# joshbeal/mira

Hardware: AMD Instinct MI355X
Metric: bn256_g1_msm_throughput (higher is better)
Workload: dtype u256 mod p (9 x 29-bit limbs in u32/u64, Montgomery)

## Files before the change

mira_amd/csrc/field29.cuh:

```cuda
#pragma once
#include "field.cuh"

struct Fq29 {
    using Sat = FqP;
    static constexpr uint32_t P[9] = {0x187cfd47u, 0x010460b6u, 0x1c72a34fu, 0x02d522d0u, 0x1585d978u, 0x02db40c0u, 0x00a6e141u, 0x0e5c2634u, 0x0030644eu};
    static constexpr uint32_t N0 = 0x04866389u;
    static constexpr uint32_t ONE[9] = {0x157ccc21u, 0x141c2758u, 0x185230d3u, 0x014c0419u, 0x0aa36fb9u, 0x1d4240ceu, 0x11d54c07u, 0x052ac7a8u, 0x000dc836u};
    static constexpr uint32_t R256_TO_R261[9] = {0x13349ca1u, 0x1a5d84a8u, 0x0a3e5cacu, 0x100249e0u, 0x12b951e8u, 0x0e92d304u, 0x14cb95b3u, 0x041b9d3du, 0x00058003u};
};
struct Fr29 {
    using Sat = FrP;
    static constexpr uint32_t P[9] = {0x10000001u, 0x1f0fac9fu, 0x0e5c2450u, 0x07d090f3u, 0x1585d283u, 0x02db40c0u, 0x00a6e141u, 0x0e5c2634u, 0x0030644eu};
    static constexpr uint32_t N0 = 0x0fffffffu;
    static constexpr uint32_t ONE[9] = {0x0fffff57u, 0x1ea70ab4u, 0x052c068bu, 0x17504f49u, 0x0aa8075bu, 0x1d4240ceu, 0x11d54c07u, 0x052ac7a8u, 0x000dc836u};
    static constexpr uint32_t R256_TO_R261[9] = {0x0fffead7u, 0x1d5444f4u, 0x04438aa5u, 0x03b4d096u, 0x134c84dau, 0x0e92d304u, 0x14cb95b3u, 0x041b9d3du, 0x00058003u};
};

static constexpr uint32_t M29 = 0x1FFFFFFFu;

#ifdef F29_TRACK
#include <cassert>
#include "f29_census.h"
#define F29_BD(x) double bd = (x);
#define F29_SET(v, x) ((v).bd = (x))
#define F29_GET(v) ((v).bd)
#define F29_ASSERT(c) assert(c)
#define F29_HIT(fn, site) emu_hit(fn, site)
#define F29_REGION(name) EMU_REGION_SCOPE(name)
#else
#define F29_BD(x)
#define F29_SET(v, x) ((void)0)
#define F29_GET(v) (0.0)
#define F29_ASSERT(c) ((void)0)
#define F29_HIT(fn, site) ((void)0)
#define F29_REGION(name) ((void)0)
#endif
static constexpr double F29_RP_OVER_P = 168.0;

template <class F> struct Fe29 {
    uint32_t l[9];
    F29_BD(0.0)
};

template <class F> HD Fe29<F> f29_zero() {
    Fe29<F> r;
#pragma unroll
    for (int i = 0; i < 9; i++) r.l[i] = 0;
    return r;
}
template <class F> HD Fe29<F> f29_one() {
    Fe29<F> r;
#pragma unroll
    for (int i = 0; i < 9; i++) r.l[i] = F::ONE[i];
    F29_SET(r, 1.0);
    return r;
}
template <class F> HD bool f29_is_literal_zero(const Fe29<F> &a) {
    uint32_t o = 0;
#pragma unroll
    for (int i = 0; i < 9; i++) o |= a.l[i];
    return o == 0;
}

template <class F> HD Fe29<F> f29_carry(const Fe29<F> &a) {
    Fe29<F> r;
    r.l[0] = a.l[0] & M29;
#pragma unroll
    for (int i = 1; i < 8; i++) r.l[i] = (a.l[i] & M29) + (a.l[i - 1] >> 29);
    r.l[8] = a.l[8] + (a.l[7] >> 29);
    F29_SET(r, F29_GET(a));
    return r;
}
template <class F> HD Fe29<F> f29_add(const Fe29<F> &a, const Fe29<F> &b) {
    Fe29<F> r;
#pragma unroll
    for (int i = 0; i < 9; i++) r.l[i] = a.l[i] + b.l[i];
    F29_SET(r, F29_GET(a) + F29_GET(b));
    F29_ASSERT(F29_GET(r) <= 40.0);
    return f29_carry(r);
}
template <class F> HD Fe29<F> f29_dbl(const Fe29<F> &a) { return f29_add(a, a); }
template <class F, int K> struct F29Bias {
    uint32_t l[9];
    constexpr F29Bias() : l{} {
        uint64_t carry = 0;
        for (int i = 0; i < 9; i++) {
            uint64_t v = (uint64_t)K * F::P[i] + carry;
            l[i] = (i < 8) ? (uint32_t)(v & M29) : (uint32_t)v;
            carry = v >> 29;
        }
        for (int i = 0; i < 8; i++) {
            l[i] += 0x80000000u;
            l[i + 1] -= 4;
        }
    }
};
template <int K, class F> HD Fe29<F> f29_sub(const Fe29<F> &a, const Fe29<F> &b) {
    constexpr F29Bias<F, K> bias{};
    Fe29<F> r;
#pragma unroll
    for (int i = 0; i < 9; i++) r.l[i] = a.l[i] + bias.l[i] - b.l[i];
    F29_ASSERT(F29_GET(b) <= (double)K - 0.01);
    F29_SET(r, F29_GET(a) + (double)K);
    F29_ASSERT(F29_GET(r) <= 40.0);
    return f29_carry(r);
}
template <int K, class F> HD Fe29<F> f29_sub_b_2c(const Fe29<F> &a, const Fe29<F> &b, const Fe29<F> &c) {
    constexpr F29Bias<F, K> bias{};
    Fe29<F> r;
#pragma unroll
    for (int i = 0; i < 9; i++) r.l[i] = a.l[i] + bias.l[i] - b.l[i] - 2u * c.l[i];
    F29_ASSERT(F29_GET(b) + 2.0 * F29_GET(c) <= (double)K - 0.01);
    F29_SET(r, F29_GET(a) + (double)K);
    F29_ASSERT(F29_GET(r) <= 40.0);
    return f29_carry(r);
}
template <int K, class F> HD Fe29<F> f29_neg(const Fe29<F> &b) { return f29_sub<K>(f29_zero<F>(), b); }
template <class F> HD Fe29<F> f29_triple(const Fe29<F> &a) { return f29_add(f29_dbl(a), a); }

template <class F> HD Fe29<F> f29_add_nc(const Fe29<F> &a, const Fe29<F> &b) {
    Fe29<F> r;
#pragma unroll
    for (int i = 0; i < 9; i++) r.l[i] = a.l[i] + b.l[i];
    F29_SET(r, F29_GET(a) + F29_GET(b));
    F29_ASSERT(F29_GET(r) <= 40.0);
    return r;
}
template <class F, int K, int RAISE = 1> struct F29BiasTight {
    uint32_t l[9];
    bool ok;
    constexpr F29BiasTight() : l{}, ok(true) {
        uint64_t carry = 0;
        for (int i = 0; i < 9; i++) {
            uint64_t v = (uint64_t)K * F::P[i] + carry;
            l[i] = (i < 8) ? (uint32_t)(v & M29) : (uint32_t)v;
            carry = v >> 29;
            if (l[i] < 8u) ok = false;
        }
        for (int i = 0; i < 8; i++) {
            l[i] += (uint32_t)RAISE * 0x20000000u;
            l[i + 1] -= (uint32_t)RAISE;
        }
    }
};
template <int K, class F, int RAISE = 1> HD Fe29<F> f29_sub_nc(const Fe29<F> &a, const Fe29<F> &b) {
    constexpr F29BiasTight<F, K, RAISE> bias{};
    static_assert(bias.ok, "a limb of K * P is too small for this bias");
    Fe29<F> r;
#pragma unroll
    for (int i = 0; i < 9; i++) {
        F29_ASSERT(b.l[i] <= bias.l[i]);
        r.l[i] = a.l[i] + bias.l[i] - b.l[i];
        F29_ASSERT(r.l[i] >= a.l[i]);
    }
    F29_ASSERT(F29_GET(b) <= (double)K - 1.0);
    F29_SET(r, F29_GET(a) + (double)K);
    F29_ASSERT(F29_GET(r) <= 40.0);
    return r;
}
#ifdef F29_TRACK
template <class F> inline void f29_check_columns(const Fe29<F> &a, const Fe29<F> &b) {
    uint32_t ma = 0, mb = 0;
    for (int i = 0; i < 9; i++) { ma = a.l[i] > ma ? a.l[i] : ma; mb = b.l[i] > mb ? b.l[i] : mb; }
    const long double col = 9.0L * (long double)ma * (long double)mb + 9.0L * 536870912.0L * 536870912.0L + 68719476736.0L;
    assert(col < 18446744073709551616.0L);
}
template <class F> inline void f29_check_columns2(const Fe29<F> &a, const Fe29<F> &b, const Fe29<F> &c, const Fe29<F> &d) {
    uint32_t m[4] = {0, 0, 0, 0};
    const Fe29<F> *v[4] = {&a, &b, &c, &d};
    for (int k = 0; k < 4; k++)
        for (int i = 0; i < 9; i++) m[k] = v[k]->l[i] > m[k] ? v[k]->l[i] : m[k];
    const long double col = 9.0L * ((long double)m[0] * m[1] + (long double)m[2] * m[3]) + 9.0L * 536870912.0L * 536870912.0L + 68719476736.0L;
    assert(col < 18446744073709551616.0L);
}
#define F29_CHECK_COLUMNS(a, b) f29_check_columns(a, b)
#define F29_CHECK_COLUMNS2(a, b, c, d) f29_check_columns2(a, b, c, d)
#else
#define F29_CHECK_COLUMNS(a, b) ((void)0)
#define F29_CHECK_COLUMNS2(a, b, c, d) ((void)0)
#endif

template <class F> HD Fe29<F> f29_mul(const Fe29<F> &a, const Fe29<F> &b) {
    F29_ASSERT(F29_GET(a) * F29_GET(b) <= F29_RP_OVER_P);
    F29_CHECK_COLUMNS(a, b);
    uint64_t c[18];
#pragma unroll
    for (int k = 0; k < 18; k++) c[k] = 0;
#pragma unroll
    for (int i = 0; i < 9; i++)
#pragma unroll
        for (int j = 0; j < 9; j++) c[i + j] += (uint64_t)a.l[i] * b.l[j];
#pragma unroll
    for (int k = 0; k < 9; k++) {
        uint32_t m = ((uint32_t)c[k] * F::N0) & M29;
#pragma unroll
        for (int j = 0; j < 9; j++) c[k + j] += (uint64_t)m * F::P[j];
        c[k + 1] += c[k] >> 29;
    }
    Fe29<F> r;
#pragma unroll
    for (int i = 9; i < 17; i++) {
        r.l[i - 9] = (uint32_t)c[i] & M29;
        c[i + 1] += c[i] >> 29;
    }
    r.l[8] = (uint32_t)c[17];
    F29_SET(r, F29_GET(a) * F29_GET(b) / 168.9 + 1.0);
    return r;
}
template <class F> HD Fe29<F> f29_mul2_add(const Fe29<F> &a, const Fe29<F> &b, const Fe29<F> &c2, const Fe29<F> &d) {
    F29_ASSERT(F29_GET(a) * F29_GET(b) + F29_GET(c2) * F29_GET(d) <= F29_RP_OVER_P);
    F29_CHECK_COLUMNS2(a, b, c2, d);
    uint64_t c[18];
#pragma unroll
    for (int k = 0; k < 18; k++) c[k] = 0;
#pragma unroll
    for (int i = 0; i < 9; i++)
#pragma unroll
        for (int j = 0; j < 9; j++) c[i + j] += (uint64_t)a.l[i] * b.l[j];
#pragma unroll
    for (int i = 0; i < 9; i++)
#pragma unroll
        for (int j = 0; j < 9; j++) c[i + j] += (uint64_t)c2.l[i] * d.l[j];
#pragma unroll
    for (int k = 0; k < 9; k++) {
        uint32_t m = ((uint32_t)c[k] * F::N0) & M29;
#pragma unroll
        for (int j = 0; j < 9; j++) c[k + j] += (uint64_t)m * F::P[j];
        c[k + 1] += c[k] >> 29;
    }
    Fe29<F> r;
#pragma unroll
    for (int i = 9; i < 17; i++) {
        r.l[i - 9] = (uint32_t)c[i] & M29;
        c[i + 1] += c[i] >> 29;
    }
    r.l[8] = (uint32_t)c[17];
    F29_SET(r, (F29_GET(a) * F29_GET(b) + F29_GET(c2) * F29_GET(d)) / 168.9 + 1.0);
    return r;
}
template <class F> HD Fe29<F> f29_redc(const Fe29<F> &a) {
    uint64_t c[18];
#pragma unroll
    for (int k = 0; k < 9; k++) { c[k] = a.l[k]; c[k + 9] = 0; }
#pragma unroll
    for (int k = 0; k < 9; k++) {
        uint32_t m = ((uint32_t)c[k] * F::N0) & M29;
#pragma unroll
        for (int j = 0; j < 9; j++) c[k + j] += (uint64_t)m * F::P[j];
        c[k + 1] += c[k] >> 29;
    }
    Fe29<F> r;
#pragma unroll
    for (int i = 9; i < 17; i++) {
        r.l[i - 9] = (uint32_t)c[i] & M29;
        c[i + 1] += c[i] >> 29;
    }
    r.l[8] = (uint32_t)c[17];
    F29_SET(r, F29_GET(a) / 168.9 + 1.0);
    return r;
}
template <class F> HD Fe29<F> f29_sqr(const Fe29<F> &a) {
    F29_ASSERT(F29_GET(a) * F29_GET(a) <= F29_RP_OVER_P);
    uint64_t c[18];
#pragma unroll
    for (int k = 0; k < 18; k++) c[k] = 0;
    uint32_t d[9];
#pragma unroll
    for (int i = 0; i < 9; i++) d[i] = a.l[i] << 1;
#pragma unroll
    for (int i = 0; i < 9; i++) {
        c[2 * i] += (uint64_t)a.l[i] * a.l[i];
#pragma unroll
        for (int j = i + 1; j < 9; j++) c[i + j] += (uint64_t)a.l[i] * d[j];
    }
#pragma unroll
    for (int k = 0; k < 9; k++) {
        uint32_t m = ((uint32_t)c[k] * F::N0) & M29;
#pragma unroll
        for (int j = 0; j < 9; j++) c[k + j] += (uint64_t)m * F::P[j];
        c[k + 1] += c[k] >> 29;
    }
    Fe29<F> r;
#pragma unroll
    for (int i = 9; i < 17; i++) {
        r.l[i - 9] = (uint32_t)c[i] & M29;
        c[i + 1] += c[i] >> 29;
    }
    r.l[8] = (uint32_t)c[17];
    F29_SET(r, F29_GET(a) * F29_GET(a) / 168.9 + 1.0);
    return r;
}

constexpr uint32_t f29_inv_mod_2_29(uint32_t p0) {
    uint32_t x = p0;
    for (int i = 0; i < 5; i++) x *= 2u - p0 * x;
    return x & M29;
}
template <int KMAX, class F> HD bool f29_is_zero_mod_p(const Fe29<F> &a) {
    F29_ASSERT(F29_GET(a) <= (double)KMAX);
    constexpr uint32_t PINV = f29_inv_mod_2_29(F::P[0]);
    static_assert(((F::P[0] * PINV) & M29) == 1u, "P[0]^-1 mod 2^29");
    const bool maybe = ((a.l[0] * PINV) & M29) <= (uint32_t)KMAX;
    if (!maybe) return false;
    uint32_t n[9];
    uint32_t carry = 0;
#pragma unroll
    for (int i = 0; i < 8; i++) {
        uint32_t v = a.l[i] + carry;
        n[i] = v & M29;
        carry = v >> 29;
    }
    n[8] = a.l[8] + carry;
    for (uint32_t k = 0; k <= KMAX; k++) {
        uint64_t cy = 0;
        bool eq = true;
#pragma unroll
        for (int i = 0; i < 9; i++) {
            cy += (uint64_t)k * F::P[i];
            uint32_t want = (i < 8) ? (uint32_t)(cy & M29) : (uint32_t)cy;
            cy >>= 29;
            eq &= (n[i] == want);
        }
        if (eq) return true;
    }
    return false;
}

template <class F> HD Fe29<F> f29_unpack(const Fe<typename F::Sat> &s) {
    Fe29<F> r;
    r.l[0] = s.l[0] & M29;
    r.l[1] = ((s.l[0] >> 29) | (s.l[1] << 3)) & M29;
    r.l[2] = ((s.l[1] >> 26) | (s.l[2] << 6)) & M29;
    r.l[3] = ((s.l[2] >> 23) | (s.l[3] << 9)) & M29;
    r.l[4] = ((s.l[3] >> 20) | (s.l[4] << 12)) & M29;
    r.l[5] = ((s.l[4] >> 17) | (s.l[5] << 15)) & M29;
    r.l[6] = ((s.l[5] >> 14) | (s.l[6] << 18)) & M29;
    r.l[7] = ((s.l[6] >> 11) | (s.l[7] << 21)) & M29;
    r.l[8] = s.l[7] >> 8;
    F29_SET(r, 6.0);
    return r;
}
template <class F> HD Fe29<F> f29_unpack_canonical(const Fe<typename F::Sat> &s) {
    Fe29<F> r = f29_unpack<F>(s);
    F29_SET(r, 1.0);
    return r;
}
template <class F> HD Fe<typename F::Sat> f29_pack(const Fe29<F> &a) {
    uint32_t n[9];
    uint32_t carry = 0;
#pragma unroll
    for (int i = 0; i < 8; i++) {
        uint32_t v = a.l[i] + carry;
        n[i] = v & M29;
        carry = v >> 29;
    }
    n[8] = a.l[8] + carry;
    Fe<typename F::Sat> s;
    s.l[0] = n[0] | (n[1] << 29);
    s.l[1] = (n[1] >> 3) | (n[2] << 26);
    s.l[2] = (n[2] >> 6) | (n[3] << 23);
    s.l[3] = (n[3] >> 9) | (n[4] << 20);
    s.l[4] = (n[4] >> 12) | (n[5] << 17);
    s.l[5] = (n[5] >> 15) | (n[6] << 14);
    s.l[6] = (n[6] >> 18) | (n[7] << 11);
    s.l[7] = (n[7] >> 21) | (n[8] << 8);
    return s;
}
template <class F> HD Fe<typename F::Sat> f29_pack_product(const Fe29<F> &a) {
#pragma unroll
    for (int i = 0; i < 8; i++) F29_ASSERT(a.l[i] <= M29);
    Fe<typename F::Sat> s;
    s.l[0] = a.l[0] | (a.l[1] << 29);
    s.l[1] = (a.l[1] >> 3) | (a.l[2] << 26);
    s.l[2] = (a.l[2] >> 6) | (a.l[3] << 23);
    s.l[3] = (a.l[3] >> 9) | (a.l[4] << 20);
    s.l[4] = (a.l[4] >> 12) | (a.l[5] << 17);
    s.l[5] = (a.l[5] >> 15) | (a.l[6] << 14);
    s.l[6] = (a.l[6] >> 18) | (a.l[7] << 11);
    s.l[7] = (a.l[7] >> 21) | (a.l[8] << 8);
    return s;
}
template <class F> HD Fe29<F> f29_from_r256(const Fe<typename F::Sat> &s) {
    Fe29<F> k;
#pragma unroll
    for (int i = 0; i < 9; i++) k.l[i] = F::R256_TO_R261[i];
    F29_SET(k, 1.0);
    return f29_mul(f29_unpack_canonical<F>(s), k);
}
template <class F> HD Fe<typename F::Sat> f29_to_r256(const Fe29<F> &a) {
    Fe<typename F::Sat> r1;
#pragma unroll
    for (int i = 0; i < 8; i++) r1.l[i] = F::Sat::R1[i];
    Fe29<F> v = f29_mul(a, f29_unpack_canonical<F>(r1));
    Fe<typename F::Sat> s = f29_pack(v);
    return reduce_once(s);
}
```

mira_amd/csrc/graph_jit.hip:

```cpp
#include "ctx.h"
#include "graph_jit.hpp"
#ifndef MIRA_CPU_EMU
#include <dlfcn.h>
#include <fcntl.h>
#include <sys/stat.h>
#include <unistd.h>

#include "jit_headers.inc"
namespace graphjit {
Rtc &rtc() {
    static Rtc loaded = [] {
        Rtc r;
        for (const char *name : {"libhiprtc.so", "libhiprtc.so.7", "/opt/rocm/lib/libhiprtc.so"}) {
            r.lib = dlopen(name, RTLD_NOW | RTLD_LOCAL);
            if (r.lib) break;
        }
        if (!r.lib) { r.error = "libhiprtc.so not found: graphs stay interpreted"; return r; }
        auto sym = [&](const char *n) { void *p = dlsym(r.lib, n); if (!p) r.error = std::string("libhiprtc.so lacks ") + n; return p; };
        r.create = reinterpret_cast<decltype(r.create)>(sym("hiprtcCreateProgram"));
        r.compile = reinterpret_cast<decltype(r.compile)>(sym("hiprtcCompileProgram"));
        r.log_size = reinterpret_cast<decltype(r.log_size)>(sym("hiprtcGetProgramLogSize"));
        r.log = reinterpret_cast<decltype(r.log)>(sym("hiprtcGetProgramLog"));
        r.code_size = reinterpret_cast<decltype(r.code_size)>(sym("hiprtcGetCodeSize"));
        r.code = reinterpret_cast<decltype(r.code)>(sym("hiprtcGetCode"));
        r.destroy = reinterpret_cast<decltype(r.destroy)>(sym("hiprtcDestroyProgram"));
        return r;
    }();
    return loaded;
}
static const char *const JIT_OPTIONS[] = {"--offload-arch=gfx950", "-O3", "-std=c++17"};
std::vector<char> compile(const std::string &src, std::string &err) {
    Rtc &r = rtc();
    std::vector<char> out;
    if (!r.error.empty()) { err = r.error; return out; }
    void *prog = nullptr;
    if (r.create(&prog, src.c_str(), "mira_jit.hip", JIT_HDR_COUNT, const_cast<const char **>(JIT_HDR_TEXT), const_cast<const char **>(JIT_HDR_NAME)) != 0) {
        err = "hiprtcCreateProgram failed";
        return out;
    }
    const int rc = r.compile(prog, 3, const_cast<const char **>(JIT_OPTIONS));
    if (rc != 0) {
        size_t n = 0;
        (void)r.log_size(prog, &n);
        std::string log(n, 0);
        if (n > 1) (void)r.log(prog, &log[0]);
        err = "hiprtcCompileProgram failed (" + std::to_string(rc) + "): " + log.substr(0, 2000);
        (void)r.destroy(&prog);
        return out;
    }
    size_t n = 0;
    if (r.code_size(prog, &n) == 0 && n) { out.resize(n); if (r.code(prog, out.data()) != 0) out.clear(); }
    if (out.empty()) err = "hiprtcGetCode failed";
    (void)r.destroy(&prog);
    return out;
}

static std::string g_cache_dir;
static uint64_t fnv1a(const void *p, size_t n, uint64_t h = 0xcbf29ce484222325ull) {
    const unsigned char *b = static_cast<const unsigned char *>(p);
    for (size_t i = 0; i < n; i++) { h ^= b[i]; h *= 0x100000001b3ull; }
    return h;
}
static bool read_file(const std::string &path, std::vector<char> &out) {
    FILE *f = fopen(path.c_str(), "rb");
    if (!f) return false;
    struct stat sb;
    if (fstat(fileno(f), &sb) != 0 || sb.st_uid != geteuid() || (sb.st_mode & (S_IWGRP | S_IWOTH))) { fclose(f); return false; }
    out.clear();
    char buf[65536];
    size_t n;
    while ((n = fread(buf, 1, sizeof buf, f)) > 0) out.insert(out.end(), buf, buf + n);
    const bool ok = !ferror(f);
    fclose(f);
    return ok;
}
static const std::string &environment_key() {
    static const std::string key = [] {
        Rtc &r = rtc();
        uint64_t h = 0xcbf29ce484222325ull;
        for (int i = 0; i < JIT_HDR_COUNT; i++) {
            h = fnv1a(JIT_HDR_TEXT[i], strlen(JIT_HDR_TEXT[i]), h);
            h = fnv1a(JIT_HDR_NAME[i], strlen(JIT_HDR_NAME[i]), h);
        }
        std::string opts;
        for (const char *o : JIT_OPTIONS) { opts += o; opts += ' '; }
        int major = 0, minor = 0, runtime = 0;
        if (r.lib) {
            auto version = reinterpret_cast<int (*)(int *, int *)>(dlsym(r.lib, "hiprtcVersion"));
            if (version) (void)version(&major, &minor);
        }
        (void)hipRuntimeGetVersion(&runtime);
        hipDeviceProp_t prop;
        std::string arch = "unknown";
        if (hipGetDeviceProperties(&prop, g.device) == hipSuccess) arch = prop.gcnArchName;
        char buf[96];
        snprintf(buf, sizeof buf, "%016llx", (unsigned long long)h);
        return "mira-jit-2 arch " + arch + " hip " + std::to_string(runtime) + " hiprtc " + std::to_string(major) + "." + std::to_string(minor) + " headers " + buf + " options " + opts;
    }();
    return key;
}
static std::string cache_path(const std::string &src) {
    const std::string &env = environment_key();
    const uint64_t a = fnv1a(src.data(), src.size()), b = fnv1a(env.data(), env.size(), a ^ 0x9e3779b97f4a7c15ull);
    char name[64];
    snprintf(name, sizeof name, "/mira_jit_%016llx%016llx.bin", (unsigned long long)a, (unsigned long long)b);
    return g_cache_dir + name;
}
static constexpr char CACHE_MAGIC[8] = {'M', 'I', 'R', 'A', 'J', 'I', 'T', '2'};
static void code_hash(const std::vector<char> &code, uint64_t out[2]) {
    out[0] = fnv1a(code.data(), code.size());
    out[1] = fnv1a(code.data(), code.size(), 0x84222325cbf29ce4ull ^ code.size());
}
std::vector<char> cache_load(const std::string &src) {
    std::vector<char> file, code;
    if (g_cache_dir.empty() || !read_file(cache_path(src), file)) return code;
    const std::string &env = environment_key();
    size_t pos = 0;
    auto take = [&](const void *want, size_t n) { const bool ok = pos + n <= file.size() && memcmp(file.data() + pos, want, n) == 0; pos += n; return ok; };
    auto take_len = [&](uint64_t &v) { if (pos + 8 > file.size()) return false; memcpy(&v, file.data() + pos, 8); pos += 8; return true; };
    uint64_t n_env = 0, n_src = 0, n_code = 0, want[2] = {0, 0}, have[2];
    if (!take(CACHE_MAGIC, 8) || !take_len(n_env) || n_env != env.size() || !take(env.data(), env.size())) return code;
    if (!take_len(n_src) || n_src != src.size() || !take(src.data(), src.size())) return code;
    if (!take_len(n_code) || !take_len(want[0]) || !take_len(want[1]) || n_code == 0 || pos + n_code != file.size()) return code;
    code.assign(file.begin() + (long)pos, file.end());
    code_hash(code, have);
    if (have[0] != want[0] || have[1] != want[1]) code.clear();
    return code;
}
void cache_store(const std::string &src, const std::vector<char> &code) {
    if (g_cache_dir.empty() || code.empty()) return;
    const std::string path = cache_path(src), tmp = path + ".tmp" + std::to_string((unsigned long long)getpid());
    const int fd = open(tmp.c_str(), O_WRONLY | O_CREAT | O_EXCL, 0600);
    FILE *f = fd >= 0 ? fdopen(fd, "wb") : nullptr;
    if (!f) { if (fd >= 0) close(fd); return; }
    const std::string &env = environment_key();
    uint64_t hash[2];
    code_hash(code, hash);
    const uint64_t n_env = env.size(), n_src = src.size(), n_code = code.size();
    bool ok = fwrite(CACHE_MAGIC, 1, 8, f) == 8 && fwrite(&n_env, 8, 1, f) == 1 && fwrite(env.data(), 1, env.size(), f) == env.size();
    ok = ok && fwrite(&n_src, 8, 1, f) == 1 && fwrite(src.data(), 1, src.size(), f) == src.size();
    ok = ok && fwrite(&n_code, 8, 1, f) == 1 && fwrite(hash, 8, 2, f) == 2 && fwrite(code.data(), 1, code.size(), f) == code.size();
    ok = (fclose(f) == 0) && ok;
    if (!ok || rename(tmp.c_str(), path.c_str()) != 0) (void)remove(tmp.c_str());
}
}

int graph_set_cache_dir(const char *dir) {
    std::string d = dir ? dir : "";
    while (d.size() > 1 && d.back() == '/') d.pop_back();
    if (!d.empty()) {
        struct stat sb;
        if (stat(d.c_str(), &sb) != 0 || !S_ISDIR(sb.st_mode)) { set_error(d + " is not a directory"); return MIRA_E_IO; }
        if (sb.st_uid != geteuid() || (sb.st_mode & (S_IWGRP | S_IWOTH))) {
            set_error(d + " must belong to the calling user and be writable by nobody else (mode 0700 or 0755): kernels found there are executed");
            return MIRA_E_BAD_ARG;
        }
    }
    graphjit::g_cache_dir = d;
    return MIRA_OK;
}
int graph_jit_compile_check(const char *src, size_t *code_size_out) {
    if (!src) { set_error("null source"); return MIRA_E_BAD_ARG; }
    if (!graphjit::rtc().error.empty()) { set_error(graphjit::rtc().error); return MIRA_E_JIT_UNAVAILABLE; }
    std::string err;
    const std::vector<char> code = graphjit::compile(src, err);
    if (code.empty()) { set_error(err); return MIRA_E_JIT_FAILED; }
    if (code_size_out) *code_size_out = code.size();
    return MIRA_OK;
}
#else
int graph_set_cache_dir(const char *) { return MIRA_OK; }
int graph_jit_compile_check(const char *, size_t *) {
    set_error("the host emulation has no run-time compiler");
    return MIRA_E_JIT_UNAVAILABLE;
}
#endif
```

mira_amd/csrc/lookup.hip:

```cpp
#include "ctx.h"
#include "lookup_kernels.cuh"

namespace {

constexpr uint32_t INV_TOP_LANES = 256;
constexpr uint32_t INV_CHUNK_DEFAULT = 8;

uint32_t inv_chunk() { return (uint32_t)std::min<size_t>(64, std::max<size_t>(2, tuned(MIRA_TUNE_INV_CHUNK, INV_CHUNK_DEFAULT))); }

struct InvPlan {
    std::vector<uint64_t> n, G;
    uint64_t ws_elems = 0;
    InvPlan(uint64_t n0, uint32_t K) {
        n.push_back(n0);
        while (n.back() > (uint64_t)INV_TOP_LANES * K) {
            G.push_back((n.back() + K - 1) / K);
            n.push_back(G.back());
            ws_elems += 2 * G.back();
        }
    }
};

template <class F> int run_inversion(InvLevel0 lv, bool pre0_ws, uint32_t *d_err) {
    const InvPlan plan(lv.n, inv_chunk());
    const size_t pre0 = pre0_ws ? lv.n : 0;
    int rc;
    if ((rc = g.inv_ws.ensure((plan.ws_elems + pre0) * 32 + 32))) return rc;
    unsigned char *ws = reinterpret_cast<unsigned char *>(g.inv_ws.p);
    if (pre0_ws) {
        lv.pre[0] = ws;
        lv.pre[1] = ws + lv.n0 * 32;
    }
    std::vector<InvLevelN> up;
    size_t off = pre0 * 32;
    for (size_t l = 1; l < plan.n.size(); l++) {
        up.push_back(InvLevelN{ws + off, ws + off + plan.n[l] * 32, plan.n[l]});
        off += 2 * plan.n[l] * 32;
    }
    const size_t D = plan.G.size();
    for (size_t l = 0; l < D; l++) {
        const uint32_t grid = ceil_div(plan.G[l], 256);
        if (l == 0) LAUNCH((k_inv_up<F, InvLevel0, InvAcc0>), grid, 256, 0, g.stream, lv, (uint64_t)plan.G[0], up[0].vals, d_err);
        else LAUNCH((k_inv_up<F, InvLevelN, InvAccN>), grid, 256, 0, g.stream, up[l - 1], (uint64_t)plan.G[l], up[l].vals, d_err);
    }
    const size_t shmem = (2 * INV_TOP_LANES + 16) * sizeof(Fe29<F>);
    if (D == 0) LAUNCH_BARRIER_FLEX((k_inv_top<F, InvLevel0, InvAcc0>), 1, INV_TOP_LANES, shmem, g.stream, lv, d_err);
    else LAUNCH_BARRIER_FLEX((k_inv_top<F, InvLevelN, InvAccN>), 1, INV_TOP_LANES, shmem, g.stream, up[D - 1], d_err);
    for (size_t l = D; l-- > 0;) {
        const uint32_t grid = ceil_div(plan.G[l], 256);
        if (l == 0) LAUNCH((k_inv_down<F, InvLevel0, InvAcc0>), grid, 256, 0, g.stream, lv, (uint64_t)plan.G[0], (const unsigned char *)up[0].vals, d_err);
        else LAUNCH((k_inv_down<F, InvLevelN, InvAccN>), grid, 256, 0, g.stream, up[l - 1], (uint64_t)plan.G[l], (const unsigned char *)up[l].vals, d_err);
    }
    return MIRA_OK;
}

int finish(const char *stage, uint32_t *d_err) {
    uint32_t err = 0;
    tm_mark(stage);
    RT_CHECK(rt_last());
    RT_CHECK(rt_d2h(&err, d_err, sizeof err, g.stream));
    RT_CHECK(rt_sync(g.stream));
    tm_end();
    if (err & LK_ERR_NONCANONICAL) { set_error(std::string(stage) + ": an input element is not canonical (>= the modulus)"); return MIRA_E_BAD_ARG; }
    if (err & LK_ERR_TABLE_FULL) { set_error(std::string(stage) + ": hash table full (internal error)"); return MIRA_E_NO_DEVICE; }
    return MIRA_OK;
}
int begin(uint32_t **d_err) {
    int rc;
    if ((rc = g.lk_err.ensure(sizeof(uint32_t)))) return rc;
    *d_err = reinterpret_cast<uint32_t *>(g.lk_err.p);
    RT_CHECK(rt_memset(*d_err, 0, sizeof(uint32_t), g.stream));
    tm_begin();
    return MIRA_OK;
}

template <class F> int batch_invert_t(void *d_out, const void *d_in, size_t n) {
    uint32_t *d_err;
    int rc;
    if ((rc = begin(&d_err))) return rc;
    InvLevel0 lv;
    memset(&lv, 0, sizeof lv);
    lv.in[0] = lv.in[1] = reinterpret_cast<const unsigned char *>(d_in);
    lv.out[0] = lv.out[1] = lv.pre[0] = lv.pre[1] = reinterpret_cast<unsigned char *>(d_out);
    lv.n0 = lv.n = n;
    if ((rc = run_inversion<F>(lv, d_out == d_in, d_err))) return rc;
    return finish("batch_invert", d_err);
}

template <class F> int lookup_h_g_t(void *d_h, void *d_g, const void *d_l, size_t n_l, const void *d_t, const void *d_m, size_t n_t, const uint64_t r[4]) {
    uint32_t *d_err;
    int rc;
    if ((rc = begin(&d_err))) return rc;
    InvLevel0 lv;
    memset(&lv, 0, sizeof lv);
    lv.in[0] = reinterpret_cast<const unsigned char *>(d_l);
    lv.in[1] = reinterpret_cast<const unsigned char *>(d_t);
    lv.out[0] = lv.pre[0] = reinterpret_cast<unsigned char *>(d_h);
    lv.out[1] = lv.pre[1] = reinterpret_cast<unsigned char *>(d_g);
    lv.mul1 = reinterpret_cast<const unsigned char *>(d_m);
    lv.n0 = n_l;
    lv.n = n_l + n_t;
    memcpy(lv.r, r, 32);
    lv.add_r = true;
    if ((rc = run_inversion<F>(lv, false, d_err))) return rc;
    return finish("lookup_h_g", d_err);
}

template <class F> int lookup_m_t(void *d_m, const void *d_l, size_t n_l, const void *d_t, size_t n_t) {
    using S = typename F::Sat;
    uint64_t cap = 2;
    while (cap < 2 * (uint64_t)n_t) cap <<= 1;
    int rc;
    if ((rc = g.lk_owner.ensure(cap * 8)) || (rc = g.lk_first.ensure(cap * 4)) || (rc = g.lk_count.ensure(cap * 4)) || (rc = g.lk_slot.ensure((size_t)n_t * 8)))
        return rc;
    LkTable tab;
    tab.owner = reinterpret_cast<uint64_t *>(g.lk_owner.p);
    tab.first = reinterpret_cast<uint32_t *>(g.lk_first.p);
    tab.count = reinterpret_cast<uint32_t *>(g.lk_count.p);
    tab.slot_of_t = reinterpret_cast<uint64_t *>(g.lk_slot.p);
    tab.mask = cap - 1;
    tab.hash_mode = (uint32_t)tuned(MIRA_TUNE_LOOKUP_HASH, 0);
    uint32_t *d_err;
    if ((rc = begin(&d_err))) return rc;
    RT_CHECK(rt_memset(tab.owner, 0, cap * 8, g.stream));
    RT_CHECK(rt_memset(tab.first, 0xFF, cap * 4, g.stream));
    RT_CHECK(rt_memset(tab.count, 0, cap * 4, g.stream));
    const unsigned char *t = reinterpret_cast<const unsigned char *>(d_t), *l = reinterpret_cast<const unsigned char *>(d_l);
    LAUNCH(k_lk_insert<S>, ceil_div(n_t, 256), 256, 0, g.stream, t, (uint64_t)n_t, tab, d_err);
    if (n_l) LAUNCH_BARRIER_FLEX(k_lk_count<S>, std::min<uint32_t>(ceil_div(n_l, 256), 2048), 256, 0, g.stream, l, (uint64_t)n_l, t, tab, d_err);
    LAUNCH(k_lk_write_m<F>, ceil_div(n_t, 256), 256, 0, g.stream, tab, (uint64_t)n_t, reinterpret_cast<unsigned char *>(d_m));
    return finish("lookup_m", d_err);
}

}

int batch_invert_device(int field, void *d_out, const void *d_in, size_t n) {
    return field == MIRA_FIELD_FR ? batch_invert_t<Fr29>(d_out, d_in, n) : batch_invert_t<Fq29>(d_out, d_in, n);
}
int lookup_m_device(int field, void *d_m, const void *d_l, size_t n_l, const void *d_t, size_t n_t) {
    return field == MIRA_FIELD_FR ? lookup_m_t<Fr29>(d_m, d_l, n_l, d_t, n_t) : lookup_m_t<Fq29>(d_m, d_l, n_l, d_t, n_t);
}
int lookup_h_g_device(int field, void *d_h, void *d_g, const void *d_l, size_t n_l, const void *d_t, const void *d_m, size_t n_t, const uint64_t r[4]) {
    return field == MIRA_FIELD_FR ? lookup_h_g_t<Fr29>(d_h, d_g, d_l, n_l, d_t, d_m, n_t, r) : lookup_h_g_t<Fq29>(d_h, d_g, d_l, n_l, d_t, d_m, n_t, r);
}
```

Before: 703.5.

## Rewrite 29-bit Montgomery multiply as column-serial product-scanning with single accumulator

Replaces the 18-entry 64-bit column array in f29_mul, mul2_add, sqr and redc with a product-scanning (column-serial) Montgomery reduction that keeps one running 64-bit accumulator and the nine m values. An empty asm volatile after each multiply-add pins the accumulator so the compiler keeps a serial chain rather than re-materialising wide column arrays. The aim is lower VGPR pressure and better occupancy for the MSM kernels. It lengthens the dependency chain and is switched off for the JIT graph path and the lookup kernels.

```diff
diff --git a/mira_amd/csrc/field29.cuh b/mira_amd/csrc/field29.cuh
--- a/mira_amd/csrc/field29.cuh
+++ b/mira_amd/csrc/field29.cuh
@@ -180,9 +180,67 @@
 #define F29_CHECK_COLUMNS2(a, b, c, d) ((void)0)
 #endif
 
+#ifndef F29_COLUMN_HOOK
+#define F29_COLUMN_HOOK(k, v) ((void)0)
+#endif
+#ifndef F29_COLUMN_SERIAL
+#define F29_COLUMN_SERIAL 1
+#endif
+#if F29_COLUMN_SERIAL
+HD uint64_t f29_mad(uint32_t a, uint32_t b, uint64_t t) {
+    t += (uint64_t)a * b;
+#if defined(__HIP_DEVICE_COMPILE__)
+    asm volatile("" : : "v"(t));
+#endif
+    return t;
+}
+struct F29Limbs {
+    uint32_t l[9];
+    template <class F> HD explicit F29Limbs(const Fe29<F> &a) {
+#pragma unroll
+        for (int i = 0; i < 9; i++) l[i] = a.l[i];
+    }
+};
+template <class F, class Col> HD Fe29<F> f29_column_serial(Col col) {
+    uint32_t m[9];
+    uint64_t t = 0;
+    Fe29<F> r;
+#pragma unroll
+    for (int k = 0; k < 9; k++) {
+        t = col(k, t);
+#pragma unroll
+        for (int j = 0; j < k; j++) t = f29_mad(m[j], F::P[k - j], t);
+        m[k] = ((uint32_t)t * F::N0) & M29;
+        t = f29_mad(m[k], F::P[0], t);
+        F29_COLUMN_HOOK(k, t);
+        t >>= 29;
+    }
+#pragma unroll
+    for (int k = 9; k < 17; k++) {
+        t = col(k, t);
+#pragma unroll
+        for (int j = k - 8; j < 9; j++) t = f29_mad(m[j], F::P[k - j], t);
+        F29_COLUMN_HOOK(k, t);
+        r.l[k - 9] = (uint32_t)t & M29;
+        t >>= 29;
+    }
+    F29_COLUMN_HOOK(17, t);
+    r.l[8] = (uint32_t)t;
+    return r;
+}
+#endif
+
 template <class F> HD Fe29<F> f29_mul(const Fe29<F> &a, const Fe29<F> &b) {
     F29_ASSERT(F29_GET(a) * F29_GET(b) <= F29_RP_OVER_P);
     F29_CHECK_COLUMNS(a, b);
+#if F29_COLUMN_SERIAL
+    const F29Limbs x(a), y(b);
+    Fe29<F> r = f29_column_serial<F>([&](int k, uint64_t t) {
+#pragma unroll
+        for (int i = (k < 9 ? 0 : k - 8); i <= (k < 9 ? k : 8); i++) t = f29_mad(x.l[i], y.l[k - i], t);
+        return t;
+    });
+#else
     uint64_t c[18];
 #pragma unroll
     for (int k = 0; k < 18; k++) c[k] = 0;
@@ -204,12 +262,23 @@
         c[i + 1] += c[i] >> 29;
     }
     r.l[8] = (uint32_t)c[17];
+#endif
     F29_SET(r, F29_GET(a) * F29_GET(b) / 168.9 + 1.0);
     return r;
 }
 template <class F> HD Fe29<F> f29_mul2_add(const Fe29<F> &a, const Fe29<F> &b, const Fe29<F> &c2, const Fe29<F> &d) {
     F29_ASSERT(F29_GET(a) * F29_GET(b) + F29_GET(c2) * F29_GET(d) <= F29_RP_OVER_P);
     F29_CHECK_COLUMNS2(a, b, c2, d);
+#if F29_COLUMN_SERIAL
+    const F29Limbs x(a), y(b), z(c2), w(d);
+    Fe29<F> r = f29_column_serial<F>([&](int k, uint64_t t) {
+#pragma unroll
+        for (int i = (k < 9 ? 0 : k - 8); i <= (k < 9 ? k : 8); i++) t = f29_mad(x.l[i], y.l[k - i], t);
+#pragma unroll
+        for (int i = (k < 9 ? 0 : k - 8); i <= (k < 9 ? k : 8); i++) t = f29_mad(z.l[i], w.l[k - i], t);
+        return t;
+    });
+#else
     uint64_t c[18];
 #pragma unroll
     for (int k = 0; k < 18; k++) c[k] = 0;
@@ -235,10 +304,15 @@
         c[i + 1] += c[i] >> 29;
     }
     r.l[8] = (uint32_t)c[17];
+#endif
     F29_SET(r, (F29_GET(a) * F29_GET(b) + F29_GET(c2) * F29_GET(d)) / 168.9 + 1.0);
     return r;
 }
 template <class F> HD Fe29<F> f29_redc(const Fe29<F> &a) {
+#if F29_COLUMN_SERIAL
+    const F29Limbs x(a);
+    Fe29<F> r = f29_column_serial<F>([&](int k, uint64_t t) { return k < 9 ? t + x.l[k] : t; });
+#else
     uint64_t c[18];
 #pragma unroll
     for (int k = 0; k < 9; k++) { c[k] = a.l[k]; c[k + 9] = 0; }
@@ -256,11 +330,24 @@
         c[i + 1] += c[i] >> 29;
     }
     r.l[8] = (uint32_t)c[17];
+#endif
     F29_SET(r, F29_GET(a) / 168.9 + 1.0);
     return r;
 }
 template <class F> HD Fe29<F> f29_sqr(const Fe29<F> &a) {
     F29_ASSERT(F29_GET(a) * F29_GET(a) <= F29_RP_OVER_P);
+#if F29_COLUMN_SERIAL
+    const F29Limbs x(a);
+    uint32_t d[9];
+#pragma unroll
+    for (int i = 0; i < 9; i++) d[i] = x.l[i] << 1;
+    Fe29<F> r = f29_column_serial<F>([&](int k, uint64_t t) {
+#pragma unroll
+        for (int i = (k < 9 ? 0 : k - 8); 2 * i < k; i++) t = f29_mad(x.l[i], d[k - i], t);
+        if (k % 2 == 0) t = f29_mad(x.l[k / 2], x.l[k / 2], t);
+        return t;
+    });
+#else
     uint64_t c[18];
 #pragma unroll
     for (int k = 0; k < 18; k++) c[k] = 0;
@@ -287,6 +374,7 @@
         c[i + 1] += c[i] >> 29;
     }
     r.l[8] = (uint32_t)c[17];
+#endif
     F29_SET(r, F29_GET(a) * F29_GET(a) / 168.9 + 1.0);
     return r;
 }
diff --git a/mira_amd/csrc/graph_jit.hip b/mira_amd/csrc/graph_jit.hip
--- a/mira_amd/csrc/graph_jit.hip
+++ b/mira_amd/csrc/graph_jit.hip
@@ -28,7 +28,8 @@
     }();
     return loaded;
 }
-static const char *const JIT_OPTIONS[] = {"--offload-arch=gfx950", "-O3", "-std=c++17"};
+static const char *const JIT_OPTIONS[] = {"--offload-arch=gfx950", "-O3", "-std=c++17", "-DF29_COLUMN_SERIAL=0"};
+static constexpr int JIT_OPTION_COUNT = (int)(sizeof(JIT_OPTIONS) / sizeof(JIT_OPTIONS[0]));
 std::vector<char> compile(const std::string &src, std::string &err) {
     Rtc &r = rtc();
     std::vector<char> out;
@@ -38,7 +39,7 @@
         err = "hiprtcCreateProgram failed";
         return out;
     }
-    const int rc = r.compile(prog, 3, const_cast<const char **>(JIT_OPTIONS));
+    const int rc = r.compile(prog, JIT_OPTION_COUNT, const_cast<const char **>(JIT_OPTIONS));
     if (rc != 0) {
         size_t n = 0;
         (void)r.log_size(prog, &n);
diff --git a/mira_amd/csrc/lookup.hip b/mira_amd/csrc/lookup.hip
--- a/mira_amd/csrc/lookup.hip
+++ b/mira_amd/csrc/lookup.hip
@@ -1,3 +1,7 @@
+#if defined(__HIP_DEVICE_COMPILE__)
+#undef F29_COLUMN_SERIAL
+#define F29_COLUMN_SERIAL 0
+#endif
 #include "ctx.h"
 #include "lookup_kernels.cuh"
 
```

Result: faster. 759.7 (median of 6 runs) (+8.0%).
